# HoloTheDrunk/eray

Hardware: AMD Instinct MI355X
Metric: Mrays/s (higher is better)
Workload: dtype f32; 1 GPU; C2: cube.obj, 1920x1080 frame, 1920x1080 rows on rank 0, main.rs scene + material graph; step = 8 frames, each: camera rays, first-hit scan, shading + shadow rays, f32 image and PPM bytes; 8 frames in flight per launch; mesh=objects/cube.obj, triangles=12, rows_per_gpu=1080, texture=1024, parallelism=single GPU, frames_per_launch=8, ring_slots=8, camera=static (value); see moving_camera, culling=True

## Files before the change

eray_amd/csrc/capi.cpp:

```cpp
#include <hip/hip_runtime.h>

#include <algorithm>
#include <cmath>
#include <cstdarg>
#include <cstdio>
#include <cstdlib>
#include <cstring>
#include <new>
#include <cstddef>
#include <string>
#include <vector>

#include "../../include/eray_hip.h"
#include "internal.hpp"
#include "owners.hpp"
#include "rays_args.hpp"

using namespace eray::gpu;

namespace {
thread_local std::string g_thread_error;
constexpr size_t kMaxTags = 512;
constexpr uint32_t kUnionRing = 4;

// ... 949 lines not shown
                         rp->row0 + rp->rows, H);
    if (W && H &&
        (uint64_t)(H - 1) * rp->image_width + (W - 1) >= (uint64_t)rp->image_width * rp->image_height)
        return set_error(ctx, ERAY_E_OUT_OF_BOUNDS,
                         "camera size %ux%u does not fit the %ux%u engine image (Image::set panics)", W, H,
                         rp->image_width, rp->image_height);
    if (rp->out_ppm && (W != rp->image_width || H != rp->image_height))
        return set_error(ctx, ERAY_E_INVALID_ARGUMENT,
                         "fused PPM output needs camera size == image size; use eray_pack_ppm");
    if (rp->band_rows) {
        if (rp->band_rows % 4 || (rp->band_rows & (rp->band_rows - 1)) || rp->band_stride % 4 || rp->row0 % 4 ||
            rp->band_stride < rp->band_rows)
            return set_error(ctx, ERAY_E_INVALID_ARGUMENT,
                             "bands: band_rows (%u) must be a power of two >= 4, band_stride (%u) and row0 (%u) "
                             "multiples of 4, band_stride >= band_rows", rp->band_rows, rp->band_stride, rp->row0);
        const RowSpan rs = row_span(rp);
        if (rp->rows && (uint64_t)rp->row0 + (uint64_t)((rp->rows - 1) >> rs.band_shift) * rp->band_stride +
                                ((rp->rows - 1) & rs.band_mask) >= H)
            return set_error(ctx, ERAY_E_INVALID_ARGUMENT, "bands: %u local rows reach past the camera height %u",
                             rp->rows, H);
    }
    const bool cull = !general && !(rp->flags & ERAY_RENDER_BRUTE_FORCE);
    if (int st = sync_scene(ctx)) return st;
    *empty = !rp->rows || !W;
    if (*empty) return ERAY_OK;
    const bool trace_bins = general && !(rp->flags & ERAY_RENDER_BRUTE_FORCE) && ctx->binned > 0;
    bool known = true;
    if (cull || trace_bins)
        if (int st = sync_setup(ctx, W, H, row_span(rp), wait == SetupWait::kYes, &known, trace_bins)) return st;

    FrameParams& p = *out;
    std::memset(&p, 0, sizeof p);
    p.nframes = 1;
    const eray_camera& c = ctx->camera;
    p.cx = c.center[0];
    p.cy = c.center[1];
    p.cz = c.center[2];
    p.ratio = c.fov[0] / c.fov[1];
    p.z_dist = c.z_dist;
    p.cam_w = W;
    p.cam_h = H;
    p.img_w = rp->image_width;
    p.img_h = rp->image_height;
    p.row0 = rp->row0;
    p.rows = rp->rows;
    const RowSpan span = row_span(rp);
    p.band_shift = span.band_shift;
    p.band_mask = span.band_mask;
    p.band_stride = span.band_stride;
    p.out_rgb = rp->out_rgb;
    p.out_ppm = rp->out_ppm;
    p.out_face = rp->out_face;
    p.aligned = (p.img_w % 16) == 0 && (uint64_t)p.rows * p.img_w * 12u < (1ull << 32) &&
                ((reinterpret_cast<uintptr_t>(p.out_rgb) | reinterpret_cast<uintptr_t>(p.out_ppm) |
                  reinterpret_cast<uintptr_t>(p.out_face)) & 15) == 0;
    p.tris = ctx->d_hot;
    p.shade = ctx->d_shade;
    p.cull = cull ? ctx->d_cull : nullptr;
    p.objects = ctx->d_objs;
    p.lights = ctx->d_lights;
    p.nobj = (uint32_t)ctx->objects.size();
    p.nlights = (uint32_t)ctx->lights.size();
    p.max_object_tris = 0;
    for (auto& o : ctx->objects) p.max_object_tris = o.T > p.max_object_tris ? o.T : p.max_object_tris;
    p.total_tris = ctx->total_tris;
    p.lds_scene = (ctx->total_tris <= kCacheTris && p.nobj <= kCacheObjects && p.nlights <= kCacheLights) ? 1u : 0u;
// ... 298 lines not shown
    const uint64_t px = (uint64_t)rp->rows * rp->image_width;
    const uint64_t need[3] = {px * 12u, px * 3u, px * 4u};
    const uint64_t stride[3] = {r->rgb_stride, r->ppm_stride, r->face_stride};
    const void* ptr[3] = {rp->out_rgb, rp->out_ppm, rp->out_face};
    for (int k = 0; k < 3; ++k) {
        if (!ptr[k] || r->slots == 1) continue;
        if (stride[k] % 16 || stride[k] < need[k])
            return set_error(ctx, ERAY_E_INVALID_ARGUMENT,
                             "ring: output %d's slot stride %llu must be a multiple of 16 of at least %llu bytes", k,
                             (unsigned long long)stride[k], (unsigned long long)need[k]);
    }
    if (r->frames_per_launch && (r->frames_per_launch > r->slots || (r->frames_per_launch & (r->frames_per_launch - 1))))
        return set_error(ctx, ERAY_E_INVALID_ARGUMENT, "ring: frames_per_launch (%u) must be a power of two <= slots (%u)",
                         r->frames_per_launch, r->slots);
    out->slots = r->slots;
    out->rgb = r->slots > 1 ? r->rgb_stride : 0;
    out->ppm = r->slots > 1 ? r->ppm_stride : 0;
    out->face = r->slots > 1 ? r->face_stride : 0;
    uint32_t F = 1;
    if (p.aa || p.bounces || r->slots == 1) {
        F = 1;
    } else if (r->frames_per_launch) {
        F = r->frames_per_launch;
    } else {
        F = auto_frames(p.cam_w, p.rows, r->slots, p.max_object_tris > kDirectMax);
    }
    out->per_launch = F;
    return ERAY_OK;
}

FrameParams ring_frames(const FrameParams& p, const Ring& r, uint32_t f, uint32_t count) {
    FrameParams q = p;
    const uint64_t slot = f % r.slots;
    q.nframes = count;
    q.rgb_stride = r.rgb;
    q.ppm_stride = r.ppm;
    q.face_stride = r.face;
    if (q.out_rgb) q.out_rgb = reinterpret_cast<float*>(reinterpret_cast<char*>(q.out_rgb) + slot * r.rgb);
    if (q.out_ppm) q.out_ppm += slot * r.ppm;
    if (q.out_face) q.out_face = reinterpret_cast<int32_t*>(reinterpret_cast<char*>(q.out_face) + slot * r.face);
    const uint64_t ring_bytes = (uint64_t)r.slots * ((q.out_rgb ? r.rgb : 0) + (q.out_ppm ? r.ppm : 0) + (q.out_face ? r.face : 0));
    if (ring_bytes > kInfinityCacheBytes) q.launch_flags |= kLaunchRingBeyondCache;
    return q;
}

std::vector<unsigned char> ring_key(std::vector<unsigned char> key, const Ring& r) {
    append(key, r);
    return key;
}

struct StaticRing {
    eray_ctx* ctx;
    const FrameParams& p;
    const Ring& r;
    uint32_t frames;
    int plan(Plan* out) const {
        auto frame = [this](uint32_t f, uint32_t n) { return body(0, f, n); };
        return ensure_plan(ctx, ring_key(params_key(p, 0), r), frames, frame, out);
    }
    int before_chunk(uint32_t, uint32_t) const { return ERAY_OK; }
    int body(uint32_t, uint32_t f, uint32_t n) const {
        if (f % r.per_launch) return ERAY_OK;
        HIP_TRY(ctx, launch_frame(ctx, ring_frames(p, r, f, std::min(r.per_launch, n - f))));
        return ERAY_OK;
    }
    int plain(uint32_t f) const { return body(0, f, frames); }
};

int ensure_union(eray_ctx* ctx, uint32_t nobj) {
    if (ctx->d_union_acc && ctx->h_union && ctx->union_cap() >= nobj) return ERAY_OK;
    for (Event& ev : ctx->union_ev) {
        if (!ev) HIP_TRY(ctx, ev.create(hipEventDisableTiming));
        HIP_TRY(ctx, hipEventSynchronize(ev));
    }
    HIP_TRY(ctx, hipStreamSynchronize(ctx->stream));
    const uint32_t n = std::max<uint32_t>(nobj, 1u);
    HIP_TRY(ctx, ctx->d_union_acc.alloc(4 * (size_t)n));
    HIP_TRY(ctx, ctx->h_union.alloc(4 * (size_t)n * kUnionRing, hipHostMallocMapped));
    HIP_TRY(ctx, launch_union_flush(ctx->d_union_acc, n, nullptr, ctx->stream));
    for (auto& s : ctx->union_seq) s = 0;
    return ERAY_OK;
}
int finish_union(eray_ctx* ctx, const FrameSource& src, uint32_t nobj) {
    const uint32_t e = (uint32_t)(src.key % kUnionRing);
    HIP_TRY(ctx, hipEventSynchronize(ctx->union_ev[e]));
    HIP_TRY(ctx, launch_union_flush(ctx->d_union_acc, std::max(nobj, 1u),
                                    ctx->h_union.dev + (size_t)e * 4 * ctx->union_cap(), ctx->stream));
    HIP_TRY(ctx, hipEventRecord(ctx->union_ev[e], ctx->stream));
    ctx->union_seq[e] = src.key;
    ctx->union_src[e] = src;
    ctx->union_nobj[e] = nobj;
    ctx->union_gen[e] = ctx->scene_gen;
    return ERAY_OK;
}
}

// ... 3 lines not shown
    FrameParams p;
    bool empty = false;
    if (int st = prepare_render(ctx, rp, &p, &empty, SetupWait::kYes)) return st;
    if (empty) return ERAY_OK;
    Ring r;
    if (int st = make_ring(ctx, rp, p, ring, &r)) return st;
    Plan plan;
    return StaticRing{ctx, p, r, frames}.plan(&plan);
}

uint32_t eray_frames_per_launch(eray_ctx* ctx, const eray_render_params* rp, uint32_t slots) {
    if (!ctx || !rp || !slots) return 1u;
    if (rp->anti_aliasing || rp->bounces) return 1u;
    uint32_t W, H;
    eray_camera_size(&ctx->camera, &W, &H);
    bool binned = false;
    for (auto& o : ctx->objects) binned |= o.T > kDirectMax;
    return auto_frames(W, rp->rows, slots, binned);
}

int eray_render_prepare(eray_ctx* ctx, const eray_render_params* rp, uint32_t frames) {
    return eray_render_prepare_ring(ctx, rp, nullptr, frames);
}

int eray_render_frames_ring(eray_ctx* ctx, const eray_render_params* rp, const eray_frame_ring* ring, uint32_t frames,
                            float* mean_frame_ms) {
    FrameParams p;
    bool empty = false;
    if (mean_frame_ms) *mean_frame_ms = 0.0f;
    if (int st = prepare_render(ctx, rp, &p, &empty, SetupWait::kYes)) return st;
    if (empty || !frames) return ERAY_OK;
    Ring r;
    if (int st = make_ring(ctx, rp, p, ring, &r)) return st;
    const StaticRing run{ctx, p, r, frames};
    Plan plan;
    if (int st = run.plan(&plan)) return st;
    const int st = timed_frames(ctx, frames, mean_frame_ms, [&] { return replay(ctx, plan, frames, run); });
    if (!st) tag_frames(ctx, p.out_ppm, r.ppm, std::min(frames, r.slots), render_source(ctx, p, rp));
    return st;
}

int eray_render_frames(eray_ctx* ctx, const eray_render_params* rp, uint32_t frames, float* mean_frame_ms) {
    return eray_render_frames_ring(ctx, rp, nullptr, frames, mean_frame_ms);
}

int eray_time_frames_ring(eray_ctx* ctx, const eray_render_params* rp, const eray_frame_ring* ring, uint32_t frames,
                          eray_kernel_times* out) {
    if (!out) return set_error(ctx, ERAY_E_INVALID_ARGUMENT, "kernel timing: out is null");
    *out = eray_kernel_times{};
    FrameParams p;
    bool empty = false;
    if (int st = prepare_render(ctx, rp, &p, &empty, SetupWait::kYes)) return st;
    if (empty || !frames) return ERAY_OK;
    if (p.aa || p.bounces)
        return set_error(ctx, ERAY_E_UNSUPPORTED, "kernel timing: the frame kernel only (no anti-aliasing or bounces)");
    Ring r;
    if (int st = make_ring(ctx, rp, p, ring, &r)) return st;
    const uint32_t F = r.per_launch, L = std::max(1u, frames / F);
    LaunchTimers t(L, 4);
    HIP_TRY(ctx, t.create());
    std::vector<uint32_t> fill_used(L, 0u);
    for (uint32_t l = 0; l < L; ++l) {
        LaunchCtx lc = ctx->lc;
        lc.frame_t[0] = t.at(l, 0);
        lc.frame_t[1] = t.at(l, 1);
        lc.fill_t[0] = t.at(l, 2);
        lc.fill_t[1] = t.at(l, 3);
// ... 519 lines not shown
```

eray_amd/csrc/internal.hpp:

```cpp
#pragma once

#include <hip/hip_runtime.h>
#include <stdint.h>

#include <array>
#include <vector>

namespace eray {
namespace gpu {

struct __align__(16) TriHot {
    float4 q0, q1, q2;
};

struct __align__(16) TriShade {
    float4 s0, s1, s2, s3;
};

struct __align__(16) TriCull {
    float4 A;
    float4 B;
    float4 K;
    float4 T;
};
// ... 103 lines not shown
    uint32_t nobj, nlights;
    uint32_t max_object_tris;
    uint32_t total_tris;
    uint32_t lds_scene;
    uint32_t nrect;
    uint32_t total_sub;
    int32_t rects[kMaxRects][4];
    uint32_t spec_pow;
    uint32_t example_mat;
    uint32_t tiles_x;
    uint32_t bins_x;
    uint32_t bin_phase;
    const uint32_t* detail_list;
    const uint8_t* detail_occ;
    const uint32_t* detail_heavy;
    uint32_t detail_wgs;
    uint32_t fill_first;
    uint32_t separate_fill;
    uint32_t fill_cap;
    const CamState* cam_state;
    uint32_t detail_wgs_alt;
    uint32_t launch_flags;
    uint32_t aa, bounces;
    uint32_t seed_lo, seed_hi;
    TriCull* trace_cull;
    uint32_t trace_bins;
    uint32_t trace_heavy_wgs, trace_fill_wgs, trace_light_wgs;
    uint32_t nframes;
    uint32_t dev_slots;
    uint32_t dlist_stride;
    uint32_t dlist_split;
    uint64_t rgb_stride, ppm_stride, face_stride;
    uint32_t store_nt;
};

__host__ __device__ inline uint32_t band_camera_row(uint32_t row0, uint32_t band_shift, uint32_t band_mask,
                                                    uint32_t band_stride, uint32_t j) {
    return row0 + (j >> band_shift) * band_stride + (j & band_mask);
}
__host__ __device__ inline void band_local_range(uint32_t row0, uint32_t band_shift, uint32_t band_stride, int32_t y0,
                                                 int32_t y1, int32_t* lo, int32_t* hi) {
    if (band_shift >= 31) {
        *lo = y0 - (int32_t)row0;
        *hi = y1 - (int32_t)row0;
        return;
    }
    const int64_t B = (int64_t)1 << band_shift, S = band_stride, off = row0;
    auto floordiv = [](int64_t a, int64_t b) { return a >= 0 ? a / b : -((-a + b - 1) / b); };
    int64_t i = floordiv((int64_t)y0 - off, S), w = (int64_t)y0 - off - i * S;
    const int64_t l0 = w < B ? i * B + w : (i + 1) * B;
    i = floordiv((int64_t)y1 - off, S);
    w = (int64_t)y1 - off - i * S;
    const int64_t l1 = w < B ? i * B + w : i * B + B - 1;
    *lo = (int32_t)(l0 < -1 ? -1 : (l0 > 0x7fffffff ? 0x7fffffff : l0));
    *hi = (int32_t)(l1 < -1 ? -1 : (l1 > 0x7fffffff ? 0x7fffffff : l1));
}

struct SceneLdsLayout {
    uint32_t objs, lights, cull, hot, shade, bytes;
};
__host__ __device__ inline SceneLdsLayout scene_lds_layout(uint32_t nobj, uint32_t nl, uint32_t n, bool cull) {
    SceneLdsLayout L;
    L.objs = 0;
    L.lights = L.objs + nobj * (uint32_t)sizeof(ObjectDesc);
    L.cull = L.lights + nl * (uint32_t)sizeof(LightDesc);
    L.hot = L.cull + (cull ? n * (uint32_t)sizeof(TriCull) : 0u);
    L.shade = L.hot + n * (uint32_t)sizeof(TriHot);
// ... 153 lines not shown
```

eray_amd/csrc/render.hip:

```cpp
#include <hip/hip_ext.h>

#include <mutex>

#include "cull_record.hpp"
#include "device_math.hpp"
#include "glibc_cosf.hpp"
#include "internal.hpp"
#include "hit.hpp"

#ifndef ERAY_TRACE_POINT
#define ERAY_TRACE_POINT(k)
#define ERAY_TRACE_WAVE0(k)
#define ERAY_TRACE_VALUE(k, v)
#endif

namespace eray {
namespace gpu {
namespace {

using namespace eray::dev;

constexpr int kWG = 256;
constexpr int kTriTile = 256;

// ... 594 lines not shown
    const f3 C = mk3(cam.cx, cam.cy, cam.cz);
    const float xf = (float)px / (float)p.cam_w;
    const float yf = (float)y / (float)p.cam_h;
    const float vw = cam.ratio * 2.0f;
    const f3 horizontal = mk3(vw, 0.0f, 0.0f), vertical = mk3(0.0f, 2.0f, 0.0f);
    const f3 botleft = sub(sub(sub(C, divs(horizontal, 2.0f)), divs(vertical, 2.0f)),
                           mk3(0.0f, 0.0f, cam.z_dist));
    return normalize(sub(add(add(botleft, mul(horizontal, xf)), mul(vertical, yf)), C));
}


struct RowMap {
    uint32_t row0, shift, stride;
};
__device__ __forceinline__ uint32_t cam_row(const RowMap& m, uint32_t j) {
    return band_camera_row(m.row0, m.shift, 0xffffffffu >> (32u - m.shift), m.stride, j);
}

__device__ __forceinline__ Bundle make_bundle(const FrameParams& p, const RowMap& rm, uint32_t x0, uint32_t xe,
                                              uint32_t py0, uint32_t pye) {
    const float rw = __builtin_amdgcn_rcpf((float)p.cam_w), rh = __builtin_amdgcn_rcpf((float)p.cam_h);
    const float lo = 1.0f - 0x1p-20f, hi = 1.0f + 0x1p-20f;
    const uint32_t y0 = cam_row(rm, py0);
    return Bundle{((float)x0 * rw) * lo, ((float)xe * rw) * hi, ((float)y0 * rh) * lo,
                  ((float)(y0 + (pye - py0)) * rh) * hi};
}

struct FrameOut {
    float* rgb;
    uint8_t* ppm;
    int32_t* face;
    bool nt;
};
__device__ __forceinline__ FrameOut frame_out(const FrameParams& p, uint32_t fr) {
    return FrameOut{p.out_rgb ? reinterpret_cast<float*>(reinterpret_cast<char*>(p.out_rgb) + fr * p.rgb_stride) : nullptr,
                    p.out_ppm ? p.out_ppm + fr * p.ppm_stride : nullptr,
                    p.out_face ? reinterpret_cast<int32_t*>(reinterpret_cast<char*>(p.out_face) + fr * p.face_stride)
                               : nullptr,
                    p.store_nt != 0};
}

__device__ __forceinline__ float4 bg_rgb4(uint32_t phase) {
    const float a = 0.1f, b = 0.2f;
    return phase == 0 ? make_float4(a, a, b, a) : phase == 1 ? make_float4(a, b, a, a) : make_float4(b, a, a, b);
}
__device__ __forceinline__ uint4 bg_ppm16(uint32_t phase) {
    const uint32_t c01 = sat_u8(0.1f * 255.0f), c02 = sat_u8(0.2f * 255.0f);
    const uint32_t w0 = c01 | (c01 << 8) | (c02 << 16) | (c01 << 24);
    const uint32_t w1 = c01 | (c02 << 8) | (c01 << 16) | (c01 << 24);
    const uint32_t w2 = c02 | (c01 << 8) | (c01 << 16) | (c02 << 24);
    return phase == 0 ? make_uint4(w0, w1, w2, w0) : phase == 1 ? make_uint4(w1, w2, w0, w1) : make_uint4(w2, w0, w1, w2);
}

template <uint32_t kW, bool kNt = false>
__device__ __forceinline__ void fill_background(const FrameParams& p, const FrameOut& o, uint32_t x0, uint32_t py0, bool aligned,
                                                uint32_t lane) {
    if (aligned && x0 + kW <= p.cam_w && py0 + kBlkH <= p.rows) {
        constexpr uint32_t kRow4 = kW * 3 / 4;
        constexpr uint32_t kRow16 = kW * 3 / 16;
        constexpr uint32_t kFace4 = kW / 4;
        if (o.rgb) {
#pragma unroll
            for (uint32_t i = lane; i < kBlkH * kRow4; i += 64) {
                const uint32_t r = i / kRow4, c = i % kRow4;
                stream16(o.rgb, reinterpret_cast<float4*>(o.rgb + 3 * ((size_t)(py0 + r) * p.img_w + x0)) + c,
                         bg_rgb4(c % 3), kNt);
            }
        }
        if (o.ppm && lane < kBlkH * kRow16) {
            const uint32_t r = lane / kRow16, c = lane % kRow16;
            const size_t row = (size_t)(p.rows - py0 - kBlkH + r);
            stream16(o.ppm, reinterpret_cast<uint4*>(o.ppm + 3 * (row * p.img_w + x0)) + c, bg_ppm16(c % 3), kNt);
// ... 403 lines not shown
            o[1] = acc.g;
            o[2] = acc.b;
        }
        if (fo.ppm) {
            uint8_t* o = fo.ppm + 3 * ((size_t)(p.rows - 1 - py) * p.img_w + px);
            o[0] = (uint8_t)b0;
            o[1] = (uint8_t)b1;
            o[2] = (uint8_t)b2;
        }
    }
    ERAY_TRACE_WAVE0(7);
}

struct SubRect {
    int32_t sx0, sx1, sy0, sy1;
};
template <bool kDev>
__device__ __forceinline__ SubRect frame_rect(const FrameParams& p, const CamState* cs, uint32_t k) {
    if (kDev) return load_const(reinterpret_cast<const SubRect*>(cs->rects), k);
    return SubRect{p.rects[k][0], p.rects[k][1], p.rects[k][2], p.rects[k][3]};
}
template <bool kDev>
__device__ __forceinline__ uint32_t frame_nrect(const FrameParams& p, const CamState* cs) {
    return kDev ? load_const(&cs->nrect, 0) : p.nrect;
}
__device__ __forceinline__ bool inside(const SubRect& r, int32_t sx, int32_t sy) {
    return sx >= r.sx0 && sx <= r.sx1 && sy >= r.sy0 && sy <= r.sy1;
}

constexpr int kFillPace = 0x0f70;
constexpr int kFillPaceCached = 0x0f72;
constexpr int kFillPaceBeyond = 0x0f71;
template <bool kDev, bool kNt, bool kPace, bool kSgpr = true>
__device__ __forceinline__ void fill_blocks(const FrameParams& p, const FrameOut& o, const CamState* cs,
                                            const uint8_t* detail_occ, uint32_t f, uint32_t nf, uint32_t wave,
                                            uint32_t lane, bool aligned) {
    constexpr uint32_t nwaves = kWG / 64;
    if constexpr (kSgpr) wave = __builtin_amdgcn_readfirstlane(wave);
    const uint32_t nblk = p.tiles_x * ((p.rows + kBlkH - 1) / kBlkH);
    const uint32_t fstride = nf * nwaves;
    constexpr bool kFast = kPace && !kNt && kSgpr;
    BlockFill bf;
    if constexpr (kFast) bf = block_fill(p.img_w, lane);
    const uint32_t full_x = aligned ? p.cam_w / kBlkW : 0u, full_y = p.rows / kBlkH;
    uint32_t occ = 0;
    uint32_t it = 0;
    const uint32_t nrect = detail_occ ? 0u : frame_nrect<kDev>(p, cs);
    const uint32_t first = f * nwaves + wave, step_y = fstride / p.tiles_x, step_x = fstride - step_y * p.tiles_x;
    uint32_t by = first / p.tiles_x, bx = first - by * p.tiles_x;
    for (uint32_t blk = first; blk < nblk; blk += fstride, ++it) {
        if (it) {
            bx += step_x;
            by += step_y;
            if (bx >= p.tiles_x) {
                bx -= p.tiles_x;
                ++by;
            }
        }
        uint32_t mask = 0;
        if (detail_occ) {
            if ((it & 63u) == 0) {
                const uint32_t b = blk + lane * fstride;
                occ = b < nblk ? detail_occ[b] : 0u;
                asm volatile("" : "+v"(occ));
            }
            mask = (uint32_t)__builtin_amdgcn_readlane((int)occ, (int)(it & 63u));
        }
        for (uint32_t k = 0; k < nrect; ++k) {
            const SubRect r = frame_rect<kDev>(p, cs, k);
            if ((int32_t)by < r.sy0 || (int32_t)by > r.sy1) continue;
#pragma unroll
            for (int32_t i = 0; i < 4; ++i) {
                const int32_t sx = (int32_t)(4 * bx) + i;
                mask |= (sx >= r.sx0 && sx <= r.sx1) ? (1u << i) : 0u;
            }
        }
        if constexpr (kPace) __builtin_amdgcn_s_waitcnt(kNt ? kFillPace : kSgpr ? kFillPaceCached : kFillPaceBeyond);
        if (!mask) {
            if (kFast && bx < full_x && by < full_y)
                fill_block_fast<kNt>(p, o, bf, bx, by, lane);
            else
                fill_background<kBlkW, kNt>(p, o, bx * kBlkW, by * kBlkH, aligned, lane);
        } else if (mask != 0xfu) {
            for (uint32_t i = 0; i < 4; ++i)
                if (!((mask >> i) & 1u)) fill_background<kSubW, kNt>(p, o, bx * kBlkW + i * kSubW, by * kBlkH, aligned, lane);
        }
    }
}

template <bool kDev>
__device__ __forceinline__ void fill_frames(const FrameParams& p, uint32_t q, uint32_t nf, uint32_t wave, uint32_t lane,
                                            bool aligned, bool pace) {
    const uint32_t F = p.nframes, roles = max(nf, F);
    for (uint32_t v = q; v < roles; v += nf) {
        const uint32_t fr = v % F, slot = p.dev_slots ? fr : 0u;
        const uint8_t* occ = p.detail_occ ? p.detail_occ + (size_t)slot * (p.dlist_stride / 4) : nullptr;
        const FrameOut o = frame_out(p, fr);
        const uint32_t g = v / F, ng = (roles - fr + F - 1) / F;
        const CamState* cs = p.cam_state + slot;
        if (o.nt && pace)
            fill_blocks<kDev, true, true>(p, o, cs, occ, g, ng, wave, lane, aligned);
        else if (o.nt)
            fill_blocks<kDev, true, false>(p, o, cs, occ, g, ng, wave, lane, aligned);
        else if (pace && (p.launch_flags & kLaunchRingBeyondCache))
            fill_blocks<kDev, false, true, false>(p, o, cs, occ, g, ng, wave, lane, aligned);
        else if (pace)
            fill_blocks<kDev, false, true>(p, o, cs, occ, g, ng, wave, lane, aligned);
        else if (p.launch_flags & kLaunchRingBeyondCache)
            fill_blocks<kDev, false, false, false>(p, o, cs, occ, g, ng, wave, lane, aligned);
        else
            fill_blocks<kDev, false, false>(p, o, cs, occ, g, ng, wave, lane, aligned);
    }
}

constexpr int kDenseWgs = 4;
template <bool kCull, bool kLdsTiles, int kMat, bool kLdsScene, bool kDense = false, bool kDev = false>
__global__ void __launch_bounds__(kWG, (kMat & kMatSpecPow) ? 1 : (kLdsTiles && !kDense) ? 1 : (kDense ? kDenseWgs : 3))
    frame_kernel(const ObjectDesc* h_objects, const LightDesc* h_lights, const TriCull* h_cull, const TriHot* h_tris,
                 const void* h_aux, uint32_t h_counts, uint32_t h_total_tris, uint32_t h_total_sub,
                 uint32_t h_roles, uint32_t h_band, FrameParams p) {
    const uint32_t grid = h_roles & 0xfffu;
    uint32_t detail_wgs = (h_roles >> 12) & 0xfffu;
    bool fill_first = (h_roles >> 30) & 1u;
    const bool separate_fill = (h_roles >> 31) & 1u;
    constexpr size_t kTileBytes = (kCull && kLdsTiles) ? 0 : kTriTile * sizeof(TriHot);
    constexpr size_t kBinBytes = (kCull && kLdsTiles) ? (kWG / 64) * kBinLdsBytes + 2 * (kWG / 64) * 4 : 0;
    __shared__ __attribute__((aligned(16))) char s_large[kLdsTiles ? (kTileBytes > kBinBytes ? kTileBytes : kBinBytes) : 16];
    TriHot* s_hot = reinterpret_cast<TriHot*>(s_large);
    TriCull* s_cull = nullptr;
    char* s_bins = s_large;
    __shared__ float4 s_rgb[kBlkW * kBlkH * 3 / 4];
    __shared__ uint32_t s_ppm[kBlkW * kBlkH * 3 / 4];
    extern __shared__ __attribute__((aligned(16))) char dyn[];
    const uint32_t wave = threadIdx.x >> 6, lane = threadIdx.x & 63;
    const uint32_t nwaves = kWG / 64;
    const bool aligned = p.aligned != 0;
    const uint32_t F = ((h_roles >> 24) & 63u) + 1u;
    auto cam_state = [&](uint32_t fr) { return p.cam_state + (p.dev_slots ? fr : 0u); };
    uint32_t total_max = h_total_sub;
    if (kDev) {
        total_max = 0;
        for (uint32_t fr = 0; fr < F; ++fr) total_max = max(total_max, load_const(&cam_state(fr)->total_sub, 0));
    }
    if (kDev && p.detail_wgs_alt && F * total_max > detail_wgs * nwaves) {
        detail_wgs = p.detail_wgs_alt;
        fill_first = true;
    }
    const uint32_t nd = min(detail_wgs ? detail_wgs : grid, F * ((total_max + nwaves - 1) / nwaves));
    const uint32_t bid = (fill_first && nd < grid) ? (blockIdx.x + nd) % grid : blockIdx.x;

    ERAY_TRACE_POINT(0);
    if (bid < nd) {
        const bool counted = kLdsTiles && !(p.launch_flags & kLaunchSharedDetail);
        const uint32_t heavy0 =
            (!kCull && counted && p.detail_heavy) ? load_const(p.detail_heavy, 0) : 0xffffffffu;
        const uint32_t* list_base = kLdsScene ? p.detail_list : static_cast<const uint32_t*>(h_aux);
        uint32_t e_first = 0;
        if constexpr (!kDev && !kLdsScene) {
            const uint32_t c = (bid / F) * nwaves + wave;
            e_first = vload_u32(list_base ? list_base : reinterpret_cast<const uint32_t*>(h_objects),
                                list_base && c < h_total_sub ? c : 0u);
        }
        constexpr bool kSnake = kLdsTiles;
        const RowMap rm{p.row0, h_band & 31u, h_band >> 5};
        const uint32_t nobj = h_counts & 0xffffu;
        const uint32_t roles = max(nd, F);
        for (uint32_t v = bid; v < roles; v += nd) {
            const uint32_t fr = v % F, kw = v / F, nk = (roles - fr + F - 1) / F;
            const uint32_t c0 = kw * nwaves;
            const CamState* cs = cam_state(fr);
            const uint32_t total = kDev ? load_const(&cs->total_sub, 0) : h_total_sub;
            const uint32_t slot = (kDev && p.dev_slots) ? fr : 0u;
            const uint32_t* dlist = list_base ? (kDev ? list_base + (size_t)slot * p.dlist_stride : list_base) : nullptr;
            const FrameOut fo = frame_out(p, fr);
            const ObjectDesc* objs = h_objects + (size_t)slot * nobj;
            const TriCull* culls = h_cull ? h_cull + (size_t)slot * h_total_tris : nullptr;
            const uint32_t nrect = dlist ? 0u : frame_nrect<kDev>(p, cs);
            const CamDev cam = frame_camera<kDev>(p, cs);
            const bool split = kDev && p.dlist_split && dlist;
            const uint32_t split_heavy = split ? load_const(&cs->heavy_sub, 0) : 0u;
            const uint32_t heavy = split ? (counted ? split_heavy : 0xffffffffu) : heavy0;
            auto lpos = [&](uint32_t j) {
                return split && j >= split_heavy ? p.dlist_split - 1u - (j - split_heavy) : j;
            };
            auto locate = [&](uint32_t j, int32_t& sx, int32_t& sy, bool first = false) {
                if (dlist) {
                    const uint32_t e = __builtin_amdgcn_readfirstlane((!kDev && !kLdsScene && first && v == bid)
                                                                          ? e_first
                                                                          : vload_u32(dlist, lpos(j)));
                    sx = (int32_t)(e & 0xffffu);
                    sy = (int32_t)(e >> 16);
                    return;
                }
                for (uint32_t k = 0; k < nrect; ++k) {
                    const SubRect r = frame_rect<kDev>(p, cs, k);
                    const uint32_t w = (uint32_t)(r.sx1 - r.sx0 + 1);
                    const uint32_t a = w * (uint32_t)(r.sy1 - r.sy0 + 1);
                    if (j < a) {
                        sx = r.sx0 + (int32_t)(j % w);
                        sy = r.sy0 + (int32_t)(j / w);
                        return;
                    }
                    j -= a;
                }
            };
            int32_t sx0 = 0, sy0 = 0;
            f3 d0;
            constexpr bool kGivenRay = true;
            auto first_rays = [&]() {
                if (c0 + wave < total) locate(c0 + wave, sx0, sy0, true);
                ERAY_TRACE_WAVE0(11);
                d0 = camera_dir(cam, p, (uint32_t)sx0 * kSubW + lane % kSubW, cam_row(rm, (uint32_t)sy0 * kBlkH + lane / kSubW));
                asm volatile("" : "+v"(d0.x), "+v"(d0.y), "+v"(d0.z));
            };
            auto detail = [&](const auto& sc, const uint32_t pobj, const uint32_t* pstart) {
                const uint32_t round = nk * nwaves;
                auto job = [&](uint32_t r, bool& valid, bool& coop) {
                    const bool odd = (r & 1u) && kSnake;
                    const uint32_t first = r * round + (odd ? round - nwaves - c0 : c0);
                    valid = first < total;
                    coop = first < heavy;
                    return odd ? first + (nwaves - 1 - wave) : first + wave;
                };
                uint32_t nx_e = 0, nx_lo = 0, nx_hi = 0;
                bool nx_range = false;
                for (uint32_t r = 0;; ++r) {
                    bool valid, coop;
                    const uint32_t j = job(r, valid, coop);
                    if (!valid) break;
                    const bool active = j < total;
                    int32_t sx = sx0, sy = sy0;
                    PreRange pre{0u, 0u, false};
                    const bool have_pre = pstart && r != 0 && nx_range;
                    if (r != 0 && active) {
                        if (pstart) {
                            const uint32_t e = __builtin_amdgcn_readfirstlane(nx_e);
                            sx = (int32_t)(e & 0xffffu);
                            sy = (int32_t)(e >> 16);
                        } else {
                            locate(j, sx, sy);
                        }
                    }
                    if (have_pre && active)
                        pre = PreRange{(uint32_t)__builtin_amdgcn_readfirstlane(nx_lo),
                                       (uint32_t)__builtin_amdgcn_readfirstlane(nx_hi), true};
                    bool nvalid = false, ncoop = false;
                    const uint32_t jn = job(r + 1, nvalid, ncoop);
                    const bool nactive = nvalid && jn < total && pstart;
                    if (nactive) nx_e = vload_u32(dlist, lpos(jn));
                    nx_range = false;
                    auto mid = [&]() {
                        if (!nactive) return;
                        const uint32_t e = __builtin_amdgcn_readfirstlane(nx_e);
                        const uint32_t bin = ((cam_row(rm, (e >> 16) * kBlkH) + kBinH - p.bin_phase) / kBinH) * p.bins_x +
                                             (e & 0xffffu);
                        nx_lo = vload_u32(pstart, bin);
                        nx_hi = vload_u32(pstart, bin + 1);
                        nx_range = true;
                    };
                    render_sub<kCull, kLdsTiles, kMat, kDense>(p, fo, cam, rm, sc, (uint32_t)sx * kSubW, (uint32_t)sy * kBlkH,
                                                       active, s_hot, s_cull, s_bins, s_rgb, s_ppm, aligned,
                                                       kGivenRay && r == 0, d0, coop, pre, pobj, mid);
                }
            };
            if constexpr (kLdsScene) {
                if (v != bid) __syncthreads();
                const FrameHot hf{objs, h_lights, culls, h_tris, static_cast<const TriShade*>(h_aux), h_counts, h_total_tris,
                                  h_total_sub, grid};
                const SceneLds sc = preload_scene(hf, dyn, first_rays);
                __syncthreads();
                detail(sc, ~0u, nullptr);
            } else {
                const SceneGlobal sc{p, objs, culls};
                uint32_t pobj = ~0u;
                const uint32_t* pstart = nullptr;
                if constexpr (kLdsTiles && kCull) {
                    const ObjGeom g0 = nobj ? sc.geom(0) : ObjGeom{};
                    uint32_t warm = 0;
                    if (nobj) {
                        const uint32_t* od = reinterpret_cast<const uint32_t*>(objs);
                        warm = load_const(od + 16, 0) ^ load_const(od + 32, 0);
                    }
                    if (h_counts >> 16) warm ^= load_const(reinterpret_cast<const uint32_t*>(h_lights), 0);
                    if ((h_counts >> 16) > 2u) warm ^= load_const(reinterpret_cast<const uint32_t*>(h_lights + 2), 0);
                    first_rays();
                    asm volatile("" ::"s"(warm));
                    if (dlist)
                        for (uint32_t oi = 0; oi < nobj; ++oi) {
                            const ObjGeom g = oi == 0 ? g0 : sc.geom(oi);
                            if (g.bin_start) {
                                pobj = oi;
                                pstart = g.bin_start;
                                break;
                            }
                        }
                } else {
                    first_rays();
                }
                ERAY_TRACE_WAVE0(12);
                detail(sc, pobj, pstart);
            }
        }
        ERAY_TRACE_POINT(1);
        if (nd < grid) {
            return;
        }
    }

    if (separate_fill) return;
    const uint32_t nf = min(nd < grid ? grid - nd : grid, p.fill_cap ? p.fill_cap : grid);
    const uint32_t f = nd < grid ? bid - nd : bid;
    if (f >= nf) return;
    ERAY_TRACE_POINT(2);
    const bool pace = nd != 0 && (p.detail_occ || !(p.launch_flags & kLaunchRingBeyondCache));
    fill_frames<kDev>(p, f, nf, wave, lane, aligned, pace);
    ERAY_TRACE_POINT(3);
}

template <bool kDev>
__global__ void __launch_bounds__(kWG) fill_kernel(FrameParams p) {
    fill_frames<kDev>(p, blockIdx.x, gridDim.x, threadIdx.x >> 6, threadIdx.x & 63, p.aligned != 0, true);
}

__global__ void __launch_bounds__(kWG) ceiling_fill_kernel(FrameParams p) {
    const uint32_t lane = threadIdx.x & 63, wave = threadIdx.x >> 6;
    const uint32_t tiles_x = p.img_w / kBlkW, bands = p.rows / kBlkH, nblk = tiles_x * bands;
    const uint32_t nw = gridDim.x * (kWG / 64), w = blockIdx.x * (kWG / 64) + wave;
    for (uint32_t b = w; b < nblk * p.nframes; b += nw) {
        const uint32_t fr = b / nblk, k = b - fr * nblk, bx = k % tiles_x, by = k / tiles_x;
        const FrameOut o = frame_out(p, fr);
        if (o.rgb) {
#pragma unroll
            for (uint32_t i = lane; i < kBlkH * 48u; i += 64) {
                const uint32_t r = i / 48u, c = i % 48u;
                const float4 v = bg_rgb4(c % 3u);
                stream16_pol<false>(o.rgb, 12u * ((by * kBlkH + r) * p.img_w + bx * kBlkW) + 16u * c, 0u,
                                    make_uint4(__float_as_uint(v.x), __float_as_uint(v.y), __float_as_uint(v.z),
                                               __float_as_uint(v.w)));
            }
        }
        if (o.ppm && lane < 48u) {
            const uint32_t r = lane / 12u, c = lane % 12u;
            stream16_pol<false>(o.ppm, 3u * ((p.rows - kBlkH - by * kBlkH + r) * p.img_w + bx * kBlkW) + 16u * c, 0u,
                                bg_ppm16(c % 3u));
        }
        if (o.face) {
            const uint32_t r = lane / 16u, c = lane % 16u;
            stream16_pol<false>(o.face, 4u * ((by * kBlkH + r) * p.img_w + bx * kBlkW) + 16u * c, 0u,
// ... 34 lines not shown
}

uint32_t band_word(const FrameParams& q) { return (q.band_shift & 31u) | (q.band_stride << 5); }
template <bool K>
const void* aux_arg(const FrameParams& q) {
    return K ? static_cast<const void*>(q.shade) : static_cast<const void*>(q.detail_list);
}

uint32_t device_cus() {
    static const uint32_t cus = [] {
        int dev = 0, n = 0;
        return (hipGetDevice(&dev) == hipSuccess &&
                hipDeviceGetAttribute(&n, hipDeviceAttributeMultiprocessorCount, dev) == hipSuccess && n > 0)
                   ? (uint32_t)n
                   : 256u;
    }();
    return cus;
}

constexpr uint32_t kFillWgsPerCu = 1;

template <typename... KArgs, typename... Args>
hipError_t launch_k(void (*kernel)(KArgs...), uint32_t grid, size_t dyn, hipStream_t s, const hipEvent_t (&t)[2],
                    Args... args) {
    if (t[0])
        hipExtLaunchKernelGGL(kernel, dim3(grid), dim3(kWG), (uint32_t)dyn, s, t[0], t[1], 0u, (KArgs)args...);
    else
        kernel<<<grid, kWG, dyn, s>>>(args...);
    return hipGetLastError();
}

template <bool C, bool L, int M, bool K, bool D = false, bool V = false>
hipError_t launch_frame_kernel(const FrameParams& p, uint32_t want, size_t dyn, const LaunchCtx& lc, hipStream_t s) {
    static std::mutex mu;
    static int per_cu = -1;
    static size_t per_cu_dyn = 0;
    int wg_cu;
    {
        std::lock_guard<std::mutex> lock(mu);
        if (per_cu < 0 || per_cu_dyn != dyn) {
            if (hipOccupancyMaxActiveBlocksPerMultiprocessor(&per_cu, frame_kernel<C, L, M, K, D, V>, kWG, dyn) !=
                    hipSuccess ||
                per_cu <= 0)
                per_cu = 1;
            per_cu_dyn = dyn;
        }
        wg_cu = per_cu;
    }
    const uint32_t cus = device_cus();
    const uint32_t grid = min(min(want, (uint32_t)wg_cu * cus), kMaxFrameGrid);
    const uint32_t nblk = p.nframes * p.tiles_x * ((p.rows + kBlkH - 1) / kBlkH);
    const uint32_t total_sub = p.nframes * p.total_sub;
    auto detail_wgs = [&](float share) {
        return share >= 1.0f && grid >= 2 ? grid - max(min((uint32_t)((float)grid / share), (nblk + 63) / 64), 1u)
                                          : 0u;
    };
    FrameParams q = p;
    q.detail_wgs = detail_wgs((L && D) ? 4.0f : 2.0f);
    q.fill_first = 0;
    q.detail_wgs_alt = 0;
    if (!L) {
        if (p.cam_state) {
            q.detail_wgs_alt = detail_wgs(3.0f);
        } else if (total_sub > q.detail_wgs * (kWG / 64)) {
            q.detail_wgs = detail_wgs(3.0f);
            q.fill_first = 1;
// ... 24 lines not shown
            if (lc.fill_used) *lc.fill_used = 1u;
            if ((e = hipEventRecord(lc.join, lc.side)) != hipSuccess) return e;
            return hipStreamWaitEvent(s, lc.join, 0);
        }
    }
    return launch_k(frame_kernel<C, L, M, K, D, V>, grid, dyn, s, lc.frame_t, q.objects, q.lights, q.cull, q.tris,
                    aux_arg<K>(q), q.nobj | (q.nlights << 16), q.total_tris, q.total_sub, frame_roles(grid, q), band_word(q),
                    q);
}

template <bool C, int M, bool V>
hipError_t launch_frame_cs(const FrameParams& p, uint32_t want, const LaunchCtx& lc, hipStream_t s) {
    if (p.lds_scene) {
        const size_t dyn = scene_lds_layout(p.nobj, p.nlights, p.total_tris, C).bytes;
        return launch_frame_kernel<C, false, M, true, false, V>(p, want, dyn, lc, s);
    }
    if (p.max_object_tris > kDirectMax) {
        if constexpr (!(M & kMatSpecPow)) {
            const bool dense = (p.launch_flags & kLaunchDense)     ? true
                               : (p.launch_flags & kLaunchNoDense) ? false
                                                                   : p.nframes * p.total_sub > device_cus() * (kWG / 64);
            if (dense) return launch_frame_kernel<C, true, M, false, true, V>(p, want, 0, lc, s);
        }
        return launch_frame_kernel<C, true, M, false, false, V>(p, want, 0, lc, s);
    }
    return launch_frame_kernel<C, false, M, false, false, V>(p, want, 0, lc, s);
}
}

hipError_t launch_render(const FrameParams& p_in, const LaunchCtx& lc, hipStream_t s) {
    FrameParams p = p_in;
    if (p.nframes < 1 || p.nframes > kMaxFramesPerLaunch || ((p.aa || p.bounces) && p.nframes != 1))
        return hipErrorInvalidValue;
    {
        const uint64_t px = (uint64_t)p.nframes * p.rows * p.img_w;
        const uint64_t out = px * ((p.out_rgb ? 12u : 0u) + (p.out_ppm ? 3u : 0u) + (p.out_face ? 4u : 0u));
        p.store_nt = out > kInfinityCacheBytes ? 1u : 0u;
    }
    if (p.aa || p.bounces) return launch_trace(p, lc, s);
    const uint32_t by_n = (p.rows + kBlkH - 1) / kBlkH;
    const uint32_t nblk = p.tiles_x * by_n;
    if (!nblk) return hipSuccess;
    const uint32_t want = p.nframes * (p.cam_state ? max((nblk + 3) / 4, nblk) : max((nblk + 3) / 4, (p.total_sub + 3) / 4));
    const int mat = (p.spec_pow ? kMatSpecPow : 0) | (p.example_mat ? kMatExample : 0);
    if (p.cull && p.cam_state) {
        switch (mat) {
            case 0: return launch_frame_cs<true, 0, true>(p, want, lc, s);
            case kMatSpecPow: return launch_frame_cs<true, kMatSpecPow, true>(p, want, lc, s);
            case kMatExample: return launch_frame_cs<true, kMatExample, true>(p, want, lc, s);
            default: return launch_frame_cs<true, kMatSpecPow | kMatExample, true>(p, want, lc, s);
        }
    }
    if (p.cull) {
        switch (mat) {
            case 0: return launch_frame_cs<true, 0, false>(p, want, lc, s);
            case kMatSpecPow: return launch_frame_cs<true, kMatSpecPow, false>(p, want, lc, s);
            case kMatExample: return launch_frame_cs<true, kMatExample, false>(p, want, lc, s);
            default: return launch_frame_cs<true, kMatSpecPow | kMatExample, false>(p, want, lc, s);
        }
    }
    switch (mat) {
        case 0: return launch_frame_cs<false, 0, false>(p, want, lc, s);
        case kMatSpecPow: return launch_frame_cs<false, kMatSpecPow, false>(p, want, lc, s);
        case kMatExample: return launch_frame_cs<false, kMatExample, false>(p, want, lc, s);
        default: return launch_frame_cs<false, kMatSpecPow | kMatExample, false>(p, want, lc, s);
    }
// ... 20 lines not shown
```

Baseline: 428,000 Mrays/s.

## Render several ring generations per kernel launch in untimed static ring path

When no per-frame timing is requested, frames are now grouped into batches of kGraphFrames and each launch loops over several generations of the frame ring. Each generation reuses the same work split but writes to the next set of ring slots, so the number of kernel launches per replay drops. Kernel variants that cannot loop, along with AA/bounce traces, fall back to one launch per generation on the host. The change adds generation bookkeeping to FrameParams and to the fill and render loops. The timed path keeps the old per-launch grouping, so the two paths now behave differently.

```diff
diff --git a/eray_amd/csrc/capi.cpp b/eray_amd/csrc/capi.cpp
--- a/eray_amd/csrc/capi.cpp
+++ b/eray_amd/csrc/capi.cpp
@@ -1005,6 +1005,7 @@
     FrameParams& p = *out;
     std::memset(&p, 0, sizeof p);
     p.nframes = 1;
+    p.generations = p.gen_frames = 1;
     const eray_camera& c = ctx->camera;
     p.cx = c.center[0];
     p.cy = c.center[1];
@@ -1369,7 +1370,11 @@
 FrameParams ring_frames(const FrameParams& p, const Ring& r, uint32_t f, uint32_t count) {
     FrameParams q = p;
     const uint64_t slot = f % r.slots;
-    q.nframes = count;
+    q.nframes = std::min(count, r.per_launch);
+    q.generations = (count + q.nframes - 1) / q.nframes;
+    q.gen_frames = count;
+    q.ring_slot = (uint32_t)slot;
+    q.ring_mask = r.slots - 1;
     q.rgb_stride = r.rgb;
     q.ppm_stride = r.ppm;
     q.face_stride = r.face;
@@ -1391,14 +1396,17 @@
     const FrameParams& p;
     const Ring& r;
     uint32_t frames;
+    uint32_t group = kGraphFrames;
     int plan(Plan* out) const {
         auto frame = [this](uint32_t f, uint32_t n) { return body(0, f, n); };
-        return ensure_plan(ctx, ring_key(params_key(p, 0), r), frames, frame, out);
+        std::vector<unsigned char> key = ring_key(params_key(p, 0), r);
+        append(key, group);
+        return ensure_plan(ctx, key, frames, frame, out);
     }
     int before_chunk(uint32_t, uint32_t) const { return ERAY_OK; }
     int body(uint32_t, uint32_t f, uint32_t n) const {
-        if (f % r.per_launch) return ERAY_OK;
-        HIP_TRY(ctx, launch_frame(ctx, ring_frames(p, r, f, std::min(r.per_launch, n - f))));
+        if (f % group) return ERAY_OK;
+        HIP_TRY(ctx, launch_frame(ctx, ring_frames(p, r, f, std::min(group, n - f))));
         return ERAY_OK;
     }
     int plain(uint32_t f) const { return body(0, f, frames); }
@@ -1468,7 +1476,7 @@
     if (empty || !frames) return ERAY_OK;
     Ring r;
     if (int st = make_ring(ctx, rp, p, ring, &r)) return st;
-    const StaticRing run{ctx, p, r, frames};
+    const StaticRing run{ctx, p, r, frames, mean_frame_ms ? r.per_launch : kGraphFrames};
     Plan plan;
     if (int st = run.plan(&plan)) return st;
     const int st = timed_frames(ctx, frames, mean_frame_ms, [&] { return replay(ctx, plan, frames, run); });
diff --git a/eray_amd/csrc/internal.hpp b/eray_amd/csrc/internal.hpp
--- a/eray_amd/csrc/internal.hpp
+++ b/eray_amd/csrc/internal.hpp
@@ -159,7 +159,23 @@
     uint32_t dlist_split;
     uint64_t rgb_stride, ppm_stride, face_stride;
     uint32_t store_nt;
-};
+    uint32_t generations;
+    uint32_t gen_frames;
+    uint32_t ring_slot, ring_mask;
+};
+inline FrameParams single_generation(const FrameParams& p, uint32_t g) {
+    FrameParams q = p;
+    if (p.generations <= 1) return q;
+    const int64_t ds = (int64_t)((p.ring_slot + g * p.nframes) & p.ring_mask) - (int64_t)p.ring_slot;
+    q.generations = 1;
+    q.nframes = p.gen_frames - g * p.nframes < p.nframes ? p.gen_frames - g * p.nframes : p.nframes;
+    q.gen_frames = q.nframes;
+    q.ring_slot = (p.ring_slot + g * p.nframes) & p.ring_mask;
+    if (q.out_rgb) q.out_rgb = reinterpret_cast<float*>(reinterpret_cast<char*>(q.out_rgb) + ds * (int64_t)p.rgb_stride);
+    if (q.out_ppm) q.out_ppm += ds * (int64_t)p.ppm_stride;
+    if (q.out_face) q.out_face = reinterpret_cast<int32_t*>(reinterpret_cast<char*>(q.out_face) + ds * (int64_t)p.face_stride);
+    return q;
+}
 
 __host__ __device__ inline uint32_t band_camera_row(uint32_t row0, uint32_t band_shift, uint32_t band_mask,
                                                     uint32_t band_stride, uint32_t j) {
diff --git a/eray_amd/csrc/render.hip b/eray_amd/csrc/render.hip
--- a/eray_amd/csrc/render.hip
+++ b/eray_amd/csrc/render.hip
@@ -650,12 +650,17 @@
     int32_t* face;
     bool nt;
 };
-__device__ __forceinline__ FrameOut frame_out(const FrameParams& p, uint32_t fr) {
-    return FrameOut{p.out_rgb ? reinterpret_cast<float*>(reinterpret_cast<char*>(p.out_rgb) + fr * p.rgb_stride) : nullptr,
-                    p.out_ppm ? p.out_ppm + fr * p.ppm_stride : nullptr,
-                    p.out_face ? reinterpret_cast<int32_t*>(reinterpret_cast<char*>(p.out_face) + fr * p.face_stride)
+__device__ __forceinline__ FrameOut frame_out(const FrameParams& p, uint32_t fr, uint32_t g = 0) {
+    uint64_t k = fr;
+    if (g) k += (uint64_t)(int64_t)(int32_t)(((p.ring_slot + g * p.nframes) & p.ring_mask) - p.ring_slot);
+    return FrameOut{p.out_rgb ? reinterpret_cast<float*>(reinterpret_cast<char*>(p.out_rgb) + k * p.rgb_stride) : nullptr,
+                    p.out_ppm ? p.out_ppm + k * p.ppm_stride : nullptr,
+                    p.out_face ? reinterpret_cast<int32_t*>(reinterpret_cast<char*>(p.out_face) + k * p.face_stride)
                                : nullptr,
                     p.store_nt != 0};
+}
+__device__ __forceinline__ bool generation_has(const FrameParams& p, uint32_t g, uint32_t fr) {
+    return g * p.nframes + fr < p.gen_frames;
 }
 
 __device__ __forceinline__ float4 bg_rgb4(uint32_t phase) {
@@ -1125,7 +1130,7 @@
 constexpr int kFillPaceCached = 0x0f72;
 constexpr int kFillPaceBeyond = 0x0f71;
 template <bool kDev, bool kNt, bool kPace, bool kSgpr = true>
-__device__ __forceinline__ void fill_blocks(const FrameParams& p, const FrameOut& o, const CamState* cs,
+__device__ __forceinline__ void fill_blocks(const FrameParams& p, uint32_t fr, uint32_t gens, const CamState* cs,
                                             const uint8_t* detail_occ, uint32_t f, uint32_t nf, uint32_t wave,
                                             uint32_t lane, bool aligned) {
     constexpr uint32_t nwaves = kWG / 64;
@@ -1136,77 +1141,84 @@
     BlockFill bf;
     if constexpr (kFast) bf = block_fill(p.img_w, lane);
     const uint32_t full_x = aligned ? p.cam_w / kBlkW : 0u, full_y = p.rows / kBlkH;
-    uint32_t occ = 0;
-    uint32_t it = 0;
     const uint32_t nrect = detail_occ ? 0u : frame_nrect<kDev>(p, cs);
     const uint32_t first = f * nwaves + wave, step_y = fstride / p.tiles_x, step_x = fstride - step_y * p.tiles_x;
-    uint32_t by = first / p.tiles_x, bx = first - by * p.tiles_x;
-    for (uint32_t blk = first; blk < nblk; blk += fstride, ++it) {
-        if (it) {
-            bx += step_x;
-            by += step_y;
-            if (bx >= p.tiles_x) {
-                bx -= p.tiles_x;
-                ++by;
-            }
-        }
-        uint32_t mask = 0;
-        if (detail_occ) {
-            if ((it & 63u) == 0) {
-                const uint32_t b = blk + lane * fstride;
-                occ = b < nblk ? detail_occ[b] : 0u;
-                asm volatile("" : "+v"(occ));
-            }
-            mask = (uint32_t)__builtin_amdgcn_readlane((int)occ, (int)(it & 63u));
-        }
-        for (uint32_t k = 0; k < nrect; ++k) {
-            const SubRect r = frame_rect<kDev>(p, cs, k);
-            if ((int32_t)by < r.sy0 || (int32_t)by > r.sy1) continue;
-#pragma unroll
-            for (int32_t i = 0; i < 4; ++i) {
-                const int32_t sx = (int32_t)(4 * bx) + i;
-                mask |= (sx >= r.sx0 && sx <= r.sx1) ? (1u << i) : 0u;
-            }
-        }
-        if constexpr (kPace) __builtin_amdgcn_s_waitcnt(kNt ? kFillPace : kSgpr ? kFillPaceCached : kFillPaceBeyond);
-        if (!mask) {
-            if (kFast && bx < full_x && by < full_y)
-                fill_block_fast<kNt>(p, o, bf, bx, by, lane);
-            else
-                fill_background<kBlkW, kNt>(p, o, bx * kBlkW, by * kBlkH, aligned, lane);
-        } else if (mask != 0xfu) {
-            for (uint32_t i = 0; i < 4; ++i)
-                if (!((mask >> i) & 1u)) fill_background<kSubW, kNt>(p, o, bx * kBlkW + i * kSubW, by * kBlkH, aligned, lane);
-        }
+    const uint32_t by0 = first / p.tiles_x, bx0 = first - by0 * p.tiles_x;
+    for (uint32_t g = 0;;) {
+        const FrameOut o = frame_out(p, fr, g);
+        uint32_t occ = 0;
+        uint32_t it = 0;
+        uint32_t by = by0, bx = bx0;
+        for (uint32_t blk = first; blk < nblk; blk += fstride, ++it) {
+            if (it) {
+                bx += step_x;
+                by += step_y;
+                if (bx >= p.tiles_x) {
+                    bx -= p.tiles_x;
+                    ++by;
+                }
+            }
+            uint32_t mask = 0;
+            if (detail_occ) {
+                if ((it & 63u) == 0) {
+                    const uint32_t b = blk + lane * fstride;
+                    occ = b < nblk ? detail_occ[b] : 0u;
+                    asm volatile("" : "+v"(occ));
+                }
+                mask = (uint32_t)__builtin_amdgcn_readlane((int)occ, (int)(it & 63u));
+            }
+            for (uint32_t k = 0; k < nrect; ++k) {
+                const SubRect r = frame_rect<kDev>(p, cs, k);
+                if ((int32_t)by < r.sy0 || (int32_t)by > r.sy1) continue;
+#pragma unroll
+                for (int32_t i = 0; i < 4; ++i) {
+                    const int32_t sx = (int32_t)(4 * bx) + i;
+                    mask |= (sx >= r.sx0 && sx <= r.sx1) ? (1u << i) : 0u;
+                }
+            }
+            if constexpr (kPace) __builtin_amdgcn_s_waitcnt(kNt ? kFillPace : kSgpr ? kFillPaceCached : kFillPaceBeyond);
+            if (!mask) {
+                if (kFast && bx < full_x && by < full_y)
+                    fill_block_fast<kNt>(p, o, bf, bx, by, lane);
+                else
+                    fill_background<kBlkW, kNt>(p, o, bx * kBlkW, by * kBlkH, aligned, lane);
+            } else if (mask != 0xfu) {
+                for (uint32_t i = 0; i < 4; ++i)
+                    if (!((mask >> i) & 1u)) fill_background<kSubW, kNt>(p, o, bx * kBlkW + i * kSubW, by * kBlkH, aligned, lane);
+            }
+        }
+        if (++g >= gens || !generation_has(p, g, fr)) break;
     }
 }
 
 template <bool kDev>
 __device__ __forceinline__ void fill_frames(const FrameParams& p, uint32_t q, uint32_t nf, uint32_t wave, uint32_t lane,
-                                            bool aligned, bool pace) {
+                                            bool aligned, bool pace, uint32_t gens = 1) {
     const uint32_t F = p.nframes, roles = max(nf, F);
+    const bool nt = p.store_nt != 0;
     for (uint32_t v = q; v < roles; v += nf) {
         const uint32_t fr = v % F, slot = p.dev_slots ? fr : 0u;
         const uint8_t* occ = p.detail_occ ? p.detail_occ + (size_t)slot * (p.dlist_stride / 4) : nullptr;
-        const FrameOut o = frame_out(p, fr);
         const uint32_t g = v / F, ng = (roles - fr + F - 1) / F;
         const CamState* cs = p.cam_state + slot;
-        if (o.nt && pace)
-            fill_blocks<kDev, true, true>(p, o, cs, occ, g, ng, wave, lane, aligned);
-        else if (o.nt)
-            fill_blocks<kDev, true, false>(p, o, cs, occ, g, ng, wave, lane, aligned);
+        if (nt && pace)
+            fill_blocks<kDev, true, true>(p, fr, gens, cs, occ, g, ng, wave, lane, aligned);
+        else if (nt)
+            fill_blocks<kDev, true, false>(p, fr, gens, cs, occ, g, ng, wave, lane, aligned);
         else if (pace && (p.launch_flags & kLaunchRingBeyondCache))
-            fill_blocks<kDev, false, true, false>(p, o, cs, occ, g, ng, wave, lane, aligned);
+            fill_blocks<kDev, false, true, false>(p, fr, gens, cs, occ, g, ng, wave, lane, aligned);
         else if (pace)
-            fill_blocks<kDev, false, true>(p, o, cs, occ, g, ng, wave, lane, aligned);
+            fill_blocks<kDev, false, true>(p, fr, gens, cs, occ, g, ng, wave, lane, aligned);
         else if (p.launch_flags & kLaunchRingBeyondCache)
-            fill_blocks<kDev, false, false, false>(p, o, cs, occ, g, ng, wave, lane, aligned);
+            fill_blocks<kDev, false, false, false>(p, fr, gens, cs, occ, g, ng, wave, lane, aligned);
         else
-            fill_blocks<kDev, false, false>(p, o, cs, occ, g, ng, wave, lane, aligned);
+            fill_blocks<kDev, false, false>(p, fr, gens, cs, occ, g, ng, wave, lane, aligned);
     }
 }
 
 constexpr int kDenseWgs = 4;
+template <bool kCull, bool kLdsTiles, int kMat, bool kLdsScene, bool kDense, bool kDev>
+constexpr bool kGenerations = !kDev && !kDense && !(kCull && !kLdsTiles && kMat == kMatSpecPow && !kLdsScene);
 template <bool kCull, bool kLdsTiles, int kMat, bool kLdsScene, bool kDense = false, bool kDev = false>
 __global__ void __launch_bounds__(kWG, (kMat & kMatSpecPow) ? 1 : (kLdsTiles && !kDense) ? 1 : (kDense ? kDenseWgs : 3))
     frame_kernel(const ObjectDesc* h_objects, const LightDesc* h_lights, const TriCull* h_cull, const TriHot* h_tris,
@@ -1229,6 +1241,7 @@
     const uint32_t nwaves = kWG / 64;
     const bool aligned = p.aligned != 0;
     const uint32_t F = ((h_roles >> 24) & 63u) + 1u;
+    constexpr bool kGen = kGenerations<kCull, kLdsTiles, kMat, kLdsScene, kDense, kDev>;
     auto cam_state = [&](uint32_t fr) { return p.cam_state + (p.dev_slots ? fr : 0u); };
     uint32_t total_max = h_total_sub;
     if (kDev) {
@@ -1265,7 +1278,6 @@
             const uint32_t total = kDev ? load_const(&cs->total_sub, 0) : h_total_sub;
             const uint32_t slot = (kDev && p.dev_slots) ? fr : 0u;
             const uint32_t* dlist = list_base ? (kDev ? list_base + (size_t)slot * p.dlist_stride : list_base) : nullptr;
-            const FrameOut fo = frame_out(p, fr);
             const ObjectDesc* objs = h_objects + (size_t)slot * nobj;
             const TriCull* culls = h_cull ? h_cull + (size_t)slot * h_total_tris : nullptr;
             const uint32_t nrect = dlist ? 0u : frame_nrect<kDev>(p, cs);
@@ -1315,45 +1327,49 @@
                     coop = first < heavy;
                     return odd ? first + (nwaves - 1 - wave) : first + wave;
                 };
-                uint32_t nx_e = 0, nx_lo = 0, nx_hi = 0;
-                bool nx_range = false;
-                for (uint32_t r = 0;; ++r) {
-                    bool valid, coop;
-                    const uint32_t j = job(r, valid, coop);
-                    if (!valid) break;
-                    const bool active = j < total;
-                    int32_t sx = sx0, sy = sy0;
-                    PreRange pre{0u, 0u, false};
-                    const bool have_pre = pstart && r != 0 && nx_range;
-                    if (r != 0 && active) {
-                        if (pstart) {
+                for (uint32_t g = 0;;) {
+                    const FrameOut fo = frame_out(p, fr, kGen ? g : 0u);
+                    uint32_t nx_e = 0, nx_lo = 0, nx_hi = 0;
+                    bool nx_range = false;
+                    for (uint32_t r = 0;; ++r) {
+                        bool valid, coop;
+                        const uint32_t j = job(r, valid, coop);
+                        if (!valid) break;
+                        const bool active = j < total;
+                        int32_t sx = sx0, sy = sy0;
+                        PreRange pre{0u, 0u, false};
+                        const bool have_pre = pstart && r != 0 && nx_range;
+                        if (r != 0 && active) {
+                            if (pstart) {
+                                const uint32_t e = __builtin_amdgcn_readfirstlane(nx_e);
+                                sx = (int32_t)(e & 0xffffu);
+                                sy = (int32_t)(e >> 16);
+                            } else {
+                                locate(j, sx, sy);
+                            }
+                        }
+                        if (have_pre && active)
+                            pre = PreRange{(uint32_t)__builtin_amdgcn_readfirstlane(nx_lo),
+                                           (uint32_t)__builtin_amdgcn_readfirstlane(nx_hi), true};
+                        bool nvalid = false, ncoop = false;
+                        const uint32_t jn = job(r + 1, nvalid, ncoop);
+                        const bool nactive = nvalid && jn < total && pstart;
+                        if (nactive) nx_e = vload_u32(dlist, lpos(jn));
+                        nx_range = false;
+                        auto mid = [&]() {
+                            if (!nactive) return;
                             const uint32_t e = __builtin_amdgcn_readfirstlane(nx_e);
-                            sx = (int32_t)(e & 0xffffu);
-                            sy = (int32_t)(e >> 16);
-                        } else {
-                            locate(j, sx, sy);
-                        }
+                            const uint32_t bin = ((cam_row(rm, (e >> 16) * kBlkH) + kBinH - p.bin_phase) / kBinH) * p.bins_x +
+                                                 (e & 0xffffu);
+                            nx_lo = vload_u32(pstart, bin);
+                            nx_hi = vload_u32(pstart, bin + 1);
+                            nx_range = true;
+                        };
+                        render_sub<kCull, kLdsTiles, kMat, kDense>(p, fo, cam, rm, sc, (uint32_t)sx * kSubW, (uint32_t)sy * kBlkH,
+                                                           active, s_hot, s_cull, s_bins, s_rgb, s_ppm, aligned,
+                                                           kGivenRay && r == 0, d0, coop, pre, pobj, mid);
                     }
-                    if (have_pre && active)
-                        pre = PreRange{(uint32_t)__builtin_amdgcn_readfirstlane(nx_lo),
-                                       (uint32_t)__builtin_amdgcn_readfirstlane(nx_hi), true};
-                    bool nvalid = false, ncoop = false;
-                    const uint32_t jn = job(r + 1, nvalid, ncoop);
-                    const bool nactive = nvalid && jn < total && pstart;
-                    if (nactive) nx_e = vload_u32(dlist, lpos(jn));
-                    nx_range = false;
-                    auto mid = [&]() {
-                        if (!nactive) return;
-                        const uint32_t e = __builtin_amdgcn_readfirstlane(nx_e);
-                        const uint32_t bin = ((cam_row(rm, (e >> 16) * kBlkH) + kBinH - p.bin_phase) / kBinH) * p.bins_x +
-                                             (e & 0xffffu);
-                        nx_lo = vload_u32(pstart, bin);
-                        nx_hi = vload_u32(pstart, bin + 1);
-                        nx_range = true;
-                    };
-                    render_sub<kCull, kLdsTiles, kMat, kDense>(p, fo, cam, rm, sc, (uint32_t)sx * kSubW, (uint32_t)sy * kBlkH,
-                                                       active, s_hot, s_cull, s_bins, s_rgb, s_ppm, aligned,
-                                                       kGivenRay && r == 0, d0, coop, pre, pobj, mid);
+                    if (!kGen || ++g >= p.generations || !generation_has(p, g, fr)) break;
                 }
             };
             if constexpr (kLdsScene) {
@@ -1406,7 +1422,7 @@
     if (f >= nf) return;
     ERAY_TRACE_POINT(2);
     const bool pace = nd != 0 && (p.detail_occ || !(p.launch_flags & kLaunchRingBeyondCache));
-    fill_frames<kDev>(p, f, nf, wave, lane, aligned, pace);
+    fill_frames<kDev>(p, f, nf, wave, lane, aligned, pace, kGen ? p.generations : 1u);
     ERAY_TRACE_POINT(3);
 }
 
@@ -1507,6 +1523,13 @@
 
 template <bool C, bool L, int M, bool K, bool D = false, bool V = false>
 hipError_t launch_frame_kernel(const FrameParams& p, uint32_t want, size_t dyn, const LaunchCtx& lc, hipStream_t s) {
+    if (p.generations > 1 && !kGenerations<C, L, M, K, D, V>) {
+        for (uint32_t g = 0; g < p.generations; ++g)
+            if (hipError_t e = launch_frame_kernel<C, L, M, K, D, V>(single_generation(p, g), want, dyn, lc, s);
+                e != hipSuccess)
+                return e;
+        return hipSuccess;
+    }
     static std::mutex mu;
     static int per_cu = -1;
     static size_t per_cu_dyn = 0;
@@ -1597,6 +1620,18 @@
     FrameParams p = p_in;
     if (p.nframes < 1 || p.nframes > kMaxFramesPerLaunch || ((p.aa || p.bounces) && p.nframes != 1))
         return hipErrorInvalidValue;
+    if (p.generations > 1) {
+        if (p.cam_state || p.ring_slot % p.nframes || (p.ring_mask + 1) % p.nframes || (p.ring_mask & (p.ring_mask + 1)) ||
+            p.gen_frames <= (p.generations - 1) * p.nframes || p.gen_frames > p.generations * p.nframes)
+            return hipErrorInvalidValue;
+        if (p.aa || p.bounces) {
+            for (uint32_t g = 0; g < p.generations; ++g)
+                if (hipError_t e = launch_render(single_generation(p, g), lc, s); e != hipSuccess) return e;
+            return hipSuccess;
+        }
+    } else {
+        p.generations = 1;
+    }
     {
         const uint64_t px = (uint64_t)p.nframes * p.rows * p.img_w;
         const uint64_t out = px * ((p.out_rgb ? 12u : 0u) + (p.out_ppm ? 3u : 0u) + (p.out_face ? 4u : 0u));
```

New measurement: 464,400 Mrays/s, median of 4. 8.5% higher.
